# beautifulv0id/Convex-2D-GPU-Collision-Detection

Hardware: AMD Instinct MI355X
Metric: sat_pair_tests_per_s (higher is better)
Workload: dtype f32

## Files before the change

### convex-2d-gpu-collision-detection_amd/csrc/c2d_api.hip

```cpp
#include "c2d_internal.hpp"

namespace c2d {

__global__ void workspace_stamp_kernel(unsigned long long* stamp, unsigned ticket) { atomicMax(reinterpret_cast<unsigned*>(stamp), ticket); }

void workspace_stamp_behind(c2d_ctx* ctx, hipStream_t s)
{
    if (stream_is_capturing(s)) return;
    const unsigned ticket = workspace_next_ticket(ctx);
    hipLaunchKernelGGL(workspace_stamp_kernel, dim3(1), dim3(1), 0, s, ctx->d_ws_stamps + kStampOther, ticket);
    if (hipGetLastError() != hipSuccess) {
        (void)hipStreamSynchronize(s);
        (void)hipGetLastError();
        return;
    }
    ctx->ws_expect[kStampOther] = ticket;
    workspace_tickets_on(ctx, s);
}

}

extern "C" {

int c2d_version(void) { return C2D_VERSION_MAJOR * 1000 + C2D_VERSION_MINOR; }

const char* c2d_status_string(int status)
{
    switch (status) {
    case C2D_OK: return "ok";
    case C2D_ERR_INVALID_ARG: return "invalid argument";
    case C2D_ERR_HIP: return "HIP runtime error";
    case C2D_ERR_NO_DEVICE: return "no usable device";
    case C2D_ERR_NOMEM: return "out of memory";
    case C2D_ERR_UNSUPPORTED: return "unsupported argument combination";
    case C2D_ERR_DIST: return "multi-GPU (RCCL) error";
    default: return "unknown status";
    }
}

const char* c2d_last_error(const c2d_ctx* ctx) { return ctx ? ctx->last_error.c_str() : ""; }

int c2d_device_count(int* count)
{
    if (!count) return C2D_ERR_INVALID_ARG;
    int n = 0;
    if (hipGetDeviceCount(&n) != hipSuccess) { *count = 0; return C2D_ERR_NO_DEVICE; }
    *count = n;
    return C2D_OK;
}

int c2d_ctx_create(int device, c2d_ctx** out)
{
    if (!out) return C2D_ERR_INVALID_ARG;
    *out = nullptr;
    int n = 0;
    if (hipGetDeviceCount(&n) != hipSuccess || n <= 0 || device < 0 || device >= n) return C2D_ERR_NO_DEVICE;
    c2d_ctx* ctx = new (std::nothrow) c2d_ctx();
    if (!ctx) return C2D_ERR_NOMEM;
    ctx->device = device;
    if (hipGetDeviceProperties(&ctx->prop, device) != hipSuccess) { delete ctx; return C2D_ERR_NO_DEVICE; }
    if (std::strncmp(ctx->prop.gcnArchName, "gfx950", 6) != 0) { delete ctx; return C2D_ERR_NO_DEVICE; }
    c2d::DeviceGuard g(device);
    if (!g.ok) { delete ctx; return C2D_ERR_NO_DEVICE; }
    if (hipMalloc(&ctx->d_counters, 64) != hipSuccess || hipMalloc(&ctx->d_count_words, c2d::kWorkspaceBytes) != hipSuccess ||
        hipMemset(ctx->d_count_words, 0, c2d::kWorkspaceBytes) != hipSuccess || hipMalloc(&ctx->d_bins, 32 * sizeof(float)) != hipSuccess ||
        hipHostMalloc(reinterpret_cast<void**>(&ctx->h_pinned), 64, hipHostMallocDefault) != hipSuccess ||
        hipHostMalloc(reinterpret_cast<void**>(&ctx->h_async_err), 64, hipHostMallocMapped) != hipSuccess ||
        hipHostGetDevicePointer(reinterpret_cast<void**>(&ctx->d_async_err), ctx->h_async_err, 0) != hipSuccess) {
        if (ctx->d_counters) (void)hipFree(ctx->d_counters);
        if (ctx->d_count_words) (void)hipFree(ctx->d_count_words);
        if (ctx->d_bins) (void)hipFree(ctx->d_bins);
        if (ctx->h_pinned) (void)hipHostFree(ctx->h_pinned);
        if (ctx->h_async_err) (void)hipHostFree(ctx->h_async_err);
        delete ctx;
        return C2D_ERR_NOMEM;
    }
    *ctx->h_async_err = 0;
    ctx->d_count_words2 = ctx->d_count_words + c2d::kCountWordsBytes / 8;
    ctx->d_ws_stamps = ctx->d_count_words + c2d::kWorkspaceStampsOffset / 8;
    *out = ctx;
    return C2D_OK;
}

int c2d_ctx_destroy(c2d_ctx* ctx)
{
    if (!ctx) return C2D_OK;
    c2d::DeviceGuard g(ctx->device);
    for (auto& p : ctx->d_list)
        if (p) (void)hipFree(p);
    if (ctx->d_counters) (void)hipFree(ctx->d_counters);
    if (ctx->d_count_words) (void)hipFree(ctx->d_count_words);
    if (ctx->ws_probe_stream) (void)hipStreamDestroy(ctx->ws_probe_stream);
    if (ctx->h_ws_block) (void)hipHostFree(ctx->h_ws_block);
    if (ctx->d_bins) (void)hipFree(ctx->d_bins);
    if (ctx->d_scratch) (void)hipFree(ctx->d_scratch);
    c2d_host_pipe_free(ctx->host_pipe);
    if (ctx->h_pinned) (void)hipHostFree(ctx->h_pinned);
    if (ctx->h_async_err) (void)hipHostFree(ctx->h_async_err);
    delete ctx;
    return C2D_OK;
}

int c2d_ctx_info_sized(const c2d_ctx* ctx, c2d_device_info* out, size_t out_bytes)
{
    if (!ctx || !out || out_bytes == 0) return C2D_ERR_INVALID_ARG;
    c2d_device_info di;
    std::memset(&di, 0, sizeof di);
    if (ctx->prop.name[0]) std::snprintf(di.name, sizeof di.name, "%s", ctx->prop.name);
    else std::snprintf(di.name, sizeof di.name, "gfx950 device (the runtime reports no marketing name)");
    std::snprintf(di.arch, sizeof di.arch, "%s", ctx->prop.gcnArchName);
    di.device = ctx->device;
    di.compute_units = ctx->prop.multiProcessorCount;
    di.wavefront_size = ctx->prop.warpSize;
    di.lds_bytes_per_cu = (int)ctx->prop.maxSharedMemoryPerMultiProcessor;
    di.hbm_bytes = ctx->prop.totalGlobalMem;
    if (hipDeviceGetPCIBusId(di.pci_bus_id, (int)sizeof di.pci_bus_id, ctx->device) != hipSuccess) {
        (void)hipGetLastError();
        di.pci_bus_id[0] = 0;
    }
    std::memcpy(out, &di, out_bytes < sizeof di ? out_bytes : sizeof di);
    return C2D_OK;
// ... 118 lines not shown
```

### convex-2d-gpu-collision-detection_amd/csrc/c2d_internal.hpp

```cpp
#pragma once

#include <dlfcn.h>
#include <hip/hip_runtime.h>

#include <cstdio>
#include <cstring>
#include <string>

#include "../../include/c2d.h"
#include "c2d_count.hpp"

struct c2d_host_pipe;
void c2d_host_pipe_free(c2d_host_pipe* p);

struct c2d_ctx {
    int device = 0;
    hipDeviceProp_t prop{};
    uint32_t* d_list[2] = {nullptr, nullptr};
    size_t list_capacity = 0;
    uint32_t* d_counters = nullptr;
    unsigned long long* d_count_words = nullptr;
    unsigned long long* d_count_words2 = nullptr;
    unsigned long long* d_ws_stamps = nullptr;
    float* d_bins = nullptr;
    c2d_host_pipe* host_pipe = nullptr;
    void* d_scratch = nullptr;
    size_t scratch_bytes = 0;
    uint32_t* h_pinned = nullptr;
    uint32_t* h_async_err = nullptr;
    uint32_t* d_async_err = nullptr;
    hipStream_t ws_stream = nullptr;
    unsigned long long ws_stream_id = 0;
    bool ws_ticket_pending = false;
    bool ws_outstanding = false;
    unsigned ws_ticket = 0;
    unsigned ws_expect[c2d::kStampSlots] = {};
    hipStream_t ws_probe_stream = nullptr;
    unsigned long long* h_ws_block = nullptr;
    mutable std::string last_error;
};

#define C2D_ASYNC_ERR_POLY_K 1u
#define C2D_ASYNC_ERR_PAIR_INDEX 2u


namespace c2d {

inline int fail_hip(const c2d_ctx* ctx, hipError_t e, const char* what, const char* file, int line)
{
    if (ctx) {
        char buf[512];
        std::snprintf(buf, sizeof buf, "%s failed: %s (%s:%d)", what, hipGetErrorString(e), file, line);
        ctx->last_error = buf;
    }
    return C2D_ERR_HIP;
}

inline int fail_arg(const c2d_ctx* ctx, const char* msg)
{
    if (ctx) ctx->last_error = msg;
    return C2D_ERR_INVALID_ARG;
}

#define C2D_HIP(ctx, call)                                                        \
    do {                                                                          \
        hipError_t e__ = (call);                                                  \
        if (e__ != hipSuccess) return c2d::fail_hip(ctx, e__, #call, __FILE__, __LINE__); \
    } while (0)

#define C2D_LAUNCH_CHECK(ctx)                                                     \
    do {                                                                          \
        hipError_t e__ = hipGetLastError();                                       \
        if (e__ != hipSuccess) {                                                  \
            c2d::workspace_launch_failed(ctx);                                    \
            return c2d::fail_hip(ctx, e__, "kernel launch", __FILE__, __LINE__);  \
        }                                                                         \
        c2d::workspace_launch_ok(ctx);                                            \
    } while (0)

struct DeviceGuard {
    int prev = -1;
    bool ok = true;
    explicit DeviceGuard(int dev)
    {
        if (hipGetDevice(&prev) != hipSuccess) prev = -1;
        if (prev != dev) ok = hipSetDevice(dev) == hipSuccess;
    }
    ~DeviceGuard()
    {
        if (prev >= 0) (void)hipSetDevice(prev);
    }
};

constexpr int kMaxGrid = 1 << 24;

inline bool stream_is_capturing(hipStream_t s)
{
    hipStreamCaptureStatus st = hipStreamCaptureStatusNone;
    if (hipStreamIsCapturing(s, &st) != hipSuccess) { (void)hipGetLastError(); return false; }
    return st != hipStreamCaptureStatusNone;
}

constexpr unsigned long long kUnknownStreamId = ~0ull;
using StreamGetIdFn = hipError_t (*)(hipStream_t, unsigned long long*);
inline StreamGetIdFn stream_get_id_fn()
{
    static const StreamGetIdFn fn = [] {
        void* h = dlopen("libamdhip64.so.7", RTLD_NOLOAD | RTLD_NOW);
        void* sym = h ? dlsym(h, "hipStreamGetId") : nullptr;
        if (!sym) sym = dlsym(RTLD_DEFAULT, "hipStreamGetId");
        return reinterpret_cast<StreamGetIdFn>(sym);
    }();
    return fn;
}
inline unsigned long long stream_identity(hipStream_t s)
{
    const StreamGetIdFn fn = stream_get_id_fn();
    unsigned long long id = 0;
    if (!fn) return kUnknownStreamId;
    if (fn(s, &id) != hipSuccess) { (void)hipGetLastError(); return kUnknownStreamId; }
    return id;
}

inline bool workspace_same_stream(c2d_ctx* ctx, hipStream_t s)
{
    if (ctx->ws_stream != s) return false;
    if (ctx->ws_stream_id != kUnknownStreamId) return stream_identity(s) == ctx->ws_stream_id;
    return true;
}

inline hipStream_t forgotten_stream() { return reinterpret_cast<hipStream_t>(~static_cast<uintptr_t>(0)); }

inline int workspace_acquire(c2d_ctx* ctx, hipStream_t s, bool uses)
{
    ctx->ws_ticket_pending = false;
    if (!uses || !ctx->ws_outstanding) return C2D_OK;
    if (workspace_same_stream(ctx, s)) return C2D_OK;
    if (stream_is_capturing(s)) return C2D_OK;
    if (!ctx->ws_probe_stream) {
        hipError_t e = hipStreamCreateWithFlags(&ctx->ws_probe_stream, hipStreamNonBlocking);
        if (e == hipSuccess) e = hipHostMalloc(reinterpret_cast<void**>(&ctx->h_ws_block), kWorkspaceBytes, hipHostMallocDefault);
        if (e != hipSuccess) {
            if (ctx->ws_probe_stream) { (void)hipStreamDestroy(ctx->ws_probe_stream); ctx->ws_probe_stream = nullptr; }
            return fail_hip(ctx, e, "workspace guard set-up", __FILE__, __LINE__);
        }
    }
    hipError_t e = hipMemcpyAsync(ctx->h_ws_block, ctx->d_count_words, kWorkspaceBytes, hipMemcpyDeviceToHost, ctx->ws_probe_stream);
// ... 109 lines not shown
```

### convex-2d-gpu-collision-detection_amd/csrc/c2d_mc.hip

```cpp
#include "c2d_internal.hpp"
#include "c2d_math.hpp"

namespace c2d {

#ifdef C2D_MC_STATS
__device__ unsigned long long c2d_mc_stats_words[12];
#define C2D_MC_STAT(i, v)                                                                                     \
    do {                                                                                                      \
        const unsigned long long v__ = (unsigned long long)(v);                                               \
        if ((threadIdx.x & 63) == 0 && v__) atomicAdd(&c2d_mc_stats_words[i], v__);                           \
    } while (0)
#else
#define C2D_MC_STAT(i, v) do { } while (0)
#endif

}

#include "c2d_mc_core.hpp"

#ifdef C2D_MC_CLOCK
namespace c2d {
C2D_MC_CLOCK_WORDS(c2d_mc_clock_pair);
C2D_MC_CLOCK_WORDS(c2d_mc_clock_scenes);
}
// ... 363 lines not shown
#endif
constexpr bool kParkAdaptive = C2D_MC_PARK_ADAPTIVE != 0;
C2D_DEV Scene adaptive_scene(const Scene& sc, WaveQueue& q)
{
    if constexpr (kParkAdaptive) return park_scene(sc, q);
    else return park_exact(sc, q);
}

template <bool PARKED>
C2D_DEV uint32_t wave_count_hits_plain(const Scene& sc, uint64_t seed, uint64_t scene_id, uint64_t begin, uint32_t count, const WaveQueue& wq)
{
    const uint32_t lane = threadIdx.x & 63;
    uint32_t hits = 0;
#pragma nounroll
    for (uint32_t i = 0; i < count; i += 64) {
        const bool live = i + lane < count;
        const uint64_t s = begin + i + lane;
        const uint32_t j = (uint32_t)s & 3u;
        const U4 b0 = philox_draw_block(seed, scene_id, s >> 2, 0), b1 = philox_draw_block(seed, scene_id, s >> 2, 1);
        const U4 b2 = philox_draw_block(seed, scene_id, s >> 2, 2u + (j >> 1));
        float dx, dy, o[8];
        sample_centre(sc, u4_word(b0, (int)j), u4_word(b1, (int)j), dx, dy);
        const Scene ev = load_exact(load_eval<PARKED>(sc, wq), wq);
        float hx, hy, sn, cs;
        sample_shape(ev, (j & 1u) ? b2.z : b2.x, (j & 1u) ? b2.w : b2.y, seed, scene_id, s, hx, hy, sn, cs);
        rect_from_half_extents(hx, hy, cs, sn, dx, dy, o);
        hits += (uint32_t)__popcll(__ballot(live && rect_collide(ev.robot, o)));
    }
    return hits;
}

template <bool PARKED>
struct RectPolicy {
    using Scene = c2d::Scene;
    using Queue = WaveQueue;
    static C2D_DEV bool centre_pretest(const Scene& sc, const Queue&, float dx, float dy, unsigned long long& miss_m) { return c2d::centre_pretest(sc, dx, dy, miss_m); }
    static C2D_DEV uint32_t evaluate(const Scene& sc, Queue& wq, uint32_t w2r, uint32_t w2a, float dx, float dy, uint64_t seed, uint64_t scene_id, uint64_t sample,
                                     unsigned long long live_m)
    {
        return evaluate_samples<PARKED>(sc, wq, w2r, w2a, dx, dy, seed, scene_id, sample, live_m);
    }
    static C2D_DEV uint32_t plain(const Scene& sc, uint64_t seed, uint64_t scene_id, uint64_t begin, uint32_t count, const Queue& wq)
    {
        return wave_count_hits_plain<PARKED>(sc, seed, scene_id, begin, count, wq);
    }
    static C2D_DEV uint32_t finish(const Scene&, Queue&) { return 0u; }
};

struct PairArgs {
    float robot_w, robot_h, px, py;
    Pose pose;
    StdDev sd;
    uint64_t seed, scene_id, sample_begin, n_samples;
    uint32_t chunk;
};

#ifndef C2D_MC_PAIR_WAVES
#define C2D_MC_PAIR_WAVES 5
#endif
__global__ __launch_bounds__(kMcBlock, C2D_MC_PAIR_WAVES) void mc_pair_kernel(PairArgs A, unsigned long long* __restrict__ d_hits)
{
    __shared__ WaveQueue s_queue[kWavesPerBlock];
    const uint32_t wave = __builtin_amdgcn_readfirstlane(threadIdx.x >> 6);
    const Scene sc = park_exact(make_scene(A.robot_w, A.robot_h, A.px, A.py, A.pose, A.sd), s_queue[wave]);
    const uint64_t n_chunks = (A.n_samples + A.chunk - 1) / A.chunk;
    unsigned long long total = 0;
    C2D_MC_CLOCK_START();
    for (uint64_t ch = (uint64_t)blockIdx.x * kWavesPerBlock + wave; ch < n_chunks; ch += (uint64_t)gridDim.x * kWavesPerBlock) {
        const uint64_t off = ch * A.chunk;
        const uint64_t left = A.n_samples - off;
        const uint32_t count = left < A.chunk ? (uint32_t)left : A.chunk;
        total += wave_count_hits<RectPolicy<false>>(sc, A.seed, A.scene_id, A.sample_begin + off, count, s_queue[wave]);
    }
    C2D_MC_CLOCK_STOP(c2d_mc_clock_pair);
    if ((threadIdx.x & 63) == 0 && total) atomicAdd(d_hits, total);
}

struct ScenesArgs {
    const Pose* poses;
    const StdDev* std_devs;
    const PositionWithVarAndPoseIdx* scenes;
    AdaptiveState* state;
    uint32_t* lists[2];
    uint32_t num_poses, num_std_devs;
    float robot_w, robot_h;
    uint64_t seed, scene_id_base;
    ScheduleArgs sched;
    uint32_t* hits;
    uint32_t burst_steps;
    uint32_t n_bins;
    float bins[16], acc[16];
    uint32_t* n_used;
    PoseCPVarAndPoseIdx* rows;
};

struct RectBuilder {
    using Args = ScenesArgs;
    using Policy = RectPolicy<kParkAdaptive>;
#ifdef C2D_MC_CLOCK
    static C2D_DEV unsigned long long* clock_words() { return c2d_mc_clock_scenes; }
#endif
    static C2D_DEV Scene scene(const Args& A, const PositionWithVarAndPoseIdx& row, WaveQueue& q)
    {
        uint32_t pi = (uint32_t)(int)row.pose_idx, vi = (uint32_t)(int)row.var_idx;
        pi = pi < A.num_poses ? pi : A.num_poses - 1;
        vi = vi < A.num_std_devs ? vi : A.num_std_devs - 1;
        return adaptive_scene(make_scene(A.robot_w, A.robot_h, row.x, row.y, A.poses[pi], A.std_devs[vi]), q);
    }
};

__global__ void mc_scenes_init_kernel(AdaptiveState* state, uint32_t n_scenes)
{
    AdaptiveState init{};
    init.n_active = n_scenes;
    init.identity = 1;
    *state = init;
}

#ifndef C2D_MC_ADV_WAVES
#define C2D_MC_ADV_WAVES 7
#endif
template <bool BURST>
__global__ __launch_bounds__(kMcBlock, C2D_MC_ADV_WAVES) void mc_scenes_advance_kernel(ScenesArgs A) { mc_scenes_advance_body<BURST, RectBuilder>(A); }

__global__ __launch_bounds__(256) void mc_scenes_decide_kernel(DecideArgs A)
{
    const uint32_t n_active = A.state->n_active;
    if (n_active == 0) return;
// ... 106 lines not shown
                                 float* __restrict__ out1)
{
    const size_t stride = (size_t)gridDim.x * blockDim.x;
    for (size_t i = (size_t)blockIdx.x * blockDim.x + threadIdx.x; i < n; i += stride) {
        const uint32_t bits = in[i];
        const float x = __uint_as_float(bits);
        float a = 0.0f, b = 0.0f;
        switch (fn) {
        case C2D_MATH_LOG: a = log_(x); break;
        case C2D_MATH_SINCOS: sincos_(x, a, b); break;
        case C2D_MATH_SINCOS_U32: sincos_u32(bits, a, b); break;
        case C2D_MATH_SQRT: a = sqrt_normal_range(x); break;
        case C2D_MATH_BOX_MULLER: box_muller(bits, ~bits * 2654435761u, a, b); break;
        default: break;
        }
        out0[i] = a;
        if (out1) out1[i] = b;
    }
}

constexpr uint64_t kSceneDomain = 0x5ce9e5a3c0117de5ull;

__global__ void sample_scenes_kernel(const Pose* __restrict__ poses, uint32_t num_poses,
                                     const StdDev* __restrict__ std_devs, uint32_t num_std_devs, float r_offset,
                                     float spread, uint64_t seed, uint64_t scene_id_base, size_t n,
                                     PositionWithVarAndPoseIdx* __restrict__ scenes)
{
    const size_t stride = (size_t)gridDim.x * blockDim.x;
    for (size_t g = (size_t)blockIdx.x * blockDim.x + threadIdx.x; g < n; g += stride) {
        const U4 a = philox_block(seed ^ kSceneDomain, scene_id_base + g, 0, 0);
        const U4 b = philox_block(seed ^ kSceneDomain, scene_id_base + g, 0, 1);
        const uint32_t pose_idx = a.x % num_poses;
        const uint32_t sd_idx = a.y % num_std_devs;
        const Pose pose = poses[pose_idx];
        const StdDev sd = std_devs[sd_idx];
        const float u = fma_((float)a.z, 0x1p-32f, 0x1p-33f);
        const float theta = (float)((double)u * 2 * 3.14159265358979323846);
        float nrm, unused;
        box_muller(b.x, b.y, nrm, unused);
        const float shift = nrm * ((sd.y + sd.x) / 2) * spread;
        float st, ct;
        sincos_(theta, st, ct);
        const double bx = ((double)(pose.width / 2 + r_offset) + 2.35 + (double)sd.x) + (double)shift;
        const double by = ((double)(pose.height / 2 + r_offset) + 2.35 + (double)sd.y) + (double)shift;
        PositionWithVarAndPoseIdx row;
        row.x = (float)((double)ct * bx);
        row.y = (float)((double)st * by);
        row.var_idx = (float)sd_idx;
        row.pose_idx = (float)pose_idx;
        scenes[g] = row;
    }
}

void launch_mc_scenes_init(hipStream_t s, AdaptiveState* state, uint32_t n_scenes)
{
    hipLaunchKernelGGL(mc_scenes_init_kernel, dim3(1), dim3(1), 0, s, state, n_scenes);
}

void launch_mc_scenes_decide(hipStream_t s, unsigned blocks, const DecideArgs& D)
{
    hipLaunchKernelGGL(mc_scenes_decide_kernel, dim3(blocks), dim3(256), 0, s, D);
}

int ensure_scene_lists(c2d_ctx* ctx, size_t n)
{
    if (ctx->list_capacity >= n) return C2D_OK;
    for (auto& p : ctx->d_list) {
        if (p) (void)hipFree(p);
        p = nullptr;
    }
    ctx->list_capacity = 0;
    for (auto& p : ctx->d_list) {
        hipError_t e = hipMalloc(&p, n * sizeof(uint32_t));
        if (e != hipSuccess) { ctx->last_error = "c2d_mc_scenes: workspace allocation failed"; return C2D_ERR_NOMEM; }
    }
    ctx->list_capacity = n;
    return C2D_OK;
}

}

using namespace c2d;

extern "C" {

int c2d_math_eval(c2d_ctx* ctx, int fn, const uint32_t* d_in_bits, size_t n, float* d_out0, float* d_out1, c2d_stream stream)
{
    if (!ctx) return C2D_ERR_INVALID_ARG;
    if (n == 0) return C2D_OK;
    if (!d_in_bits || !d_out0 || fn < C2D_MATH_LOG || fn > C2D_MATH_BOX_MULLER) return fail_arg(ctx, "c2d_math_eval: bad argument");
    DeviceGuard g(ctx->device);
    hipLaunchKernelGGL(math_eval_kernel, dim3(grid_for(n, 256, ctx->prop.multiProcessorCount * 8)), dim3(256), 0,
                       (hipStream_t)stream, fn, d_in_bits, n, d_out0, d_out1);
    C2D_LAUNCH_CHECK(ctx);
    return C2D_OK;
}

int c2d_philox_normals(c2d_ctx* ctx, uint64_t seed, uint64_t scene_id, uint64_t sample_begin, size_t n,
                       float* d_normals, uint32_t* d_raw, c2d_stream stream)
{
    if (!ctx) return C2D_ERR_INVALID_ARG;
    if (n == 0) return C2D_OK;
    if (!d_normals) return fail_arg(ctx, "c2d_philox_normals: NULL output");
    DeviceGuard g(ctx->device);
    hipLaunchKernelGGL(philox_normals_kernel, dim3(grid_for(n, 256, ctx->prop.multiProcessorCount * 8)), dim3(256), 0,
                       (hipStream_t)stream, seed, scene_id, sample_begin, n, d_normals, d_raw);
    C2D_LAUNCH_CHECK(ctx);
    return C2D_OK;
}

int c2d_mc_pair(c2d_ctx* ctx, float robot_w, float robot_h, const Position* pos, const Pose* pose,
                const StdDev* std_dev, uint64_t seed, uint64_t scene_id, uint64_t sample_begin, uint64_t n_samples,
                unsigned long long* d_hits, c2d_stream stream)
{
    if (!ctx) return C2D_ERR_INVALID_ARG;
    if (!pos || !pose || !std_dev || !d_hits) return fail_arg(ctx, "c2d_mc_pair: NULL argument");
    if (n_samples == 0) return C2D_OK;
    if (sample_begin + n_samples < sample_begin || sample_begin + n_samples > (1ull << 62))
        return fail_arg(ctx, "c2d_mc_pair: sample range overflows the 2^62-sample stream");
    PairArgs A;
    A.robot_w = robot_w; A.robot_h = robot_h; A.px = pos->x; A.py = pos->y;
    A.pose = *pose; A.sd = *std_dev;
    A.seed = seed; A.scene_id = scene_id; A.sample_begin = sample_begin; A.n_samples = n_samples;
    const uint64_t target_waves = (uint64_t)ctx->prop.multiProcessorCount * 32;
    uint64_t chunk = (n_samples + target_waves - 1) / target_waves;
    chunk = ((chunk + 255) / 256) * 256;
    if (chunk < 256) chunk = 256;
    if (chunk > 8192) chunk = 8192;
    A.chunk = (uint32_t)chunk;
    const uint64_t n_chunks = (n_samples + chunk - 1) / chunk;
    uint64_t blocks = (n_chunks + kWavesPerBlock - 1) / kWavesPerBlock;
    const uint64_t max_blocks = (uint64_t)ctx->prop.multiProcessorCount * 256 / kWavesPerBlock;
    if (blocks > max_blocks) blocks = max_blocks;
    DeviceGuard g(ctx->device);
    hipLaunchKernelGGL(mc_pair_kernel, dim3((unsigned)blocks), dim3(kMcBlock), 0, (hipStream_t)stream, A, d_hits);
    C2D_LAUNCH_CHECK(ctx);
    return C2D_OK;
}

int c2d_mc_scenes(c2d_ctx* ctx, const c2d_mc_scenes_args* a, c2d_stream stream)
{
    if (!ctx) return C2D_ERR_INVALID_ARG;
    if (!a) return fail_arg(ctx, "c2d_mc_scenes: NULL args");
    if (a->n_scenes != 0 && (!a->d_poses || a->num_poses == 0)) {
        if (a->total_samples) *a->total_samples = 0;
        if (a->iterations) *a->iterations = 0;
        return fail_arg(ctx, a->d_poses ? "c2d_mc_scenes: empty pose / std_dev table" : "c2d_mc_scenes: NULL argument");
    }
    ScenesArgs A;
    A.poses = a->d_poses; A.num_poses = a->num_poses; A.robot_w = a->robot_w; A.robot_h = a->robot_h;
    return run_adaptive(ctx, a, stream, A, [](bool burst, unsigned blocks, const ScenesArgs& args, hipStream_t s) {
        if (burst) hipLaunchKernelGGL(mc_scenes_advance_kernel<true>, dim3(blocks), dim3(kMcBlock), 0, s, args);
        else hipLaunchKernelGGL(mc_scenes_advance_kernel<false>, dim3(blocks), dim3(kMcBlock), 0, s, args);
    }, "c2d_mc_scenes");
}

int c2d_sample_scenes(c2d_ctx* ctx, const Pose* d_poses, uint32_t num_poses, const StdDev* d_std_devs,
                      uint32_t num_std_devs, float robot_w, float robot_h, float spread, uint64_t seed,
                      uint64_t scene_id_base, size_t n_scenes, PositionWithVarAndPoseIdx* d_scenes, c2d_stream stream)
{
    if (!ctx) return C2D_ERR_INVALID_ARG;
    if (n_scenes == 0) return C2D_OK;
    if (!d_poses || !d_std_devs || !d_scenes || num_poses == 0 || num_std_devs == 0)
        return fail_arg(ctx, "c2d_sample_scenes: NULL / empty argument");
    DeviceGuard g(ctx->device);
    const float r_offset = (robot_w + robot_h) / 4;
    hipLaunchKernelGGL(sample_scenes_kernel, dim3(grid_for(n_scenes, 256, ctx->prop.multiProcessorCount * 8)), dim3(256), 0,
                       (hipStream_t)stream, d_poses, num_poses, d_std_devs, num_std_devs, r_offset, spread, seed,
                       scene_id_base, n_scenes, d_scenes);
    C2D_LAUNCH_CHECK(ctx);
    return C2D_OK;
}

#ifdef C2D_MC_CLOCK
int c2d_debug_mc_clock(c2d_ctx* ctx, int which, unsigned long long out[4], int reset)
{
    if (!ctx || !out || which < 0 || which > 1) return C2D_ERR_INVALID_ARG;
    DeviceGuard g(ctx->device);
    C2D_HIP(ctx, hipDeviceSynchronize());
    const unsigned long long zero[4] = {};
    if (which == 0) {
        C2D_HIP(ctx, hipMemcpyFromSymbol(out, HIP_SYMBOL(c2d_mc_clock_pair), 4 * sizeof(unsigned long long)));
        if (reset) C2D_HIP(ctx, hipMemcpyToSymbol(HIP_SYMBOL(c2d_mc_clock_pair), zero, sizeof zero));
    } else {
        C2D_HIP(ctx, hipMemcpyFromSymbol(out, HIP_SYMBOL(c2d_mc_clock_scenes), 4 * sizeof(unsigned long long)));
        if (reset) C2D_HIP(ctx, hipMemcpyToSymbol(HIP_SYMBOL(c2d_mc_clock_scenes), zero, sizeof zero));
    }
    return C2D_OK;
// ... 38 lines not shown
```

### convex-2d-gpu-collision-detection_amd/csrc/c2d_mc_core.hpp

```cpp
#pragma once

#include "c2d_internal.hpp"
#include "c2d_math.hpp"
#include "c2d_wave.hpp"

#ifndef C2D_MC_STAT
#define C2D_MC_STAT(i, v) do { } while (0)
#endif

#ifdef C2D_MC_CLOCK
#define C2D_MC_CLOCK_WORDS(name) __device__ unsigned long long name[4]
struct McClockStamp {
    unsigned long long c0, r0;
    __device__ __forceinline__ McClockStamp() : c0(__builtin_amdgcn_s_memtime()), r0(__builtin_amdgcn_s_memrealtime()) {}
    __device__ __forceinline__ void stop(unsigned long long* words) const
    {
        const unsigned long long c1 = __builtin_amdgcn_s_memtime(), r1 = __builtin_amdgcn_s_memrealtime();
        if ((threadIdx.x & 63) == 0) {
            atomicAdd(&words[0], c1 - c0);
            atomicAdd(&words[1], r1 - r0);
            atomicAdd(&words[2], 1ull);
        }
    }
};
// ... 200 lines not shown
        if (cn) {
            wave_lds_sync();
            const uint32_t take = cn < 64 ? cn : 64;
            const bool live = lane < take;
            const unsigned long long live_m = take >= 64 ? ~0ull : (1ull << take) - 1;
            const uint2 e = q.cand[cn - take + (live ? lane : 0)];
            wave_lds_sync();
            cn -= take;
            const uint64_t s = begin + e.y;
            const U4 a = philox_draw_block(seed, scene_id, s >> 2, 1);
            const uint32_t jj = (uint32_t)s & 3u;
            const uint32_t aw = jj == 0 ? a.x : (jj == 1 ? a.y : (jj == 2 ? a.z : a.w));
            float dx, dy;
            C2D_MC_STAT(4, take);
            sample_centre(sc, e.x, aw, dx, dy);
            unsigned long long miss_m;
            const bool miss = P::centre_pretest(sc, wq, dx, dy, miss_m);
            const bool undecided = live && !miss;
            const unsigned long long m = live_m & ~miss_m;
            if (undecided) {
                const uint32_t slot = un + __builtin_amdgcn_mbcnt_hi((uint32_t)(m >> 32), __builtin_amdgcn_mbcnt_lo((uint32_t)m, 0u));
                q.und_c[slot] = make_float2(dx, dy);
                q.und_idx[slot] = e.y;
            }
            un += (uint32_t)__popcll(m);
        }
        if (un >= 64 || (drained && cn == 0 && un)) hits += evaluate_queued<P>(sc, wq, q.und_c, q.und_idx, un, un < 64 ? un : 64u, seed, scene_id, begin);
        if (drained && cn == 0 && un == 0) break;
    }
    return hits;
}
#endif

template <class P>
C2D_DEV uint32_t wave_count_hits(const typename P::Scene& sc, uint64_t seed, uint64_t scene_id, uint64_t begin, uint32_t count,
                                 typename P::Queue& q)
{
    C2D_MC_STAT(0, count);
    if (!sc.tame()) return P::plain(sc, seed, scene_id, begin, count, q);
#ifndef C2D_MC_NO_PRETEST
    if (sc.use_x0 && sc.x0 < kFarX0) {
        C2D_MC_STAT(1, count);
        const uint32_t h = wave_count_hits_far<P>(sc, seed, scene_id, begin, count, q) + P::finish(sc, q);
        C2D_MC_STAT(7, h);
        return h;
    }
#endif
    C2D_MC_STAT(2, count);
    const uint32_t h = wave_count_hits_near<P>(sc, seed, scene_id, begin, count, q) + P::finish(sc, q);
    C2D_MC_STAT(7, h);
    return h;
}

struct AdaptiveState {
    uint32_t n_active;
    uint32_t next_count;
    uint32_t n_samples;
    uint32_t iter;
    uint32_t ticket;
    uint32_t list_sel;
    uint32_t identity;
    uint32_t burst_steps;
    unsigned long long total_samples;
};

struct ScheduleArgs {
    uint32_t small_batch, large_batch, switch_at, max_samples;
    uint32_t want_waves;
    uint32_t min_chunk;
};

C2D_DEV uint32_t batch_of(const ScheduleArgs& S, uint32_t n_samples)
{
    return n_samples < S.switch_at ? S.small_batch : S.large_batch;
}

C2D_DEV float calc_slack(uint32_t n, uint32_t k)
{
    if (k == n || k == 0) {
        return (float)(0x1.d82d33932720dp+1 / (double)n);
    }
    const float z = 1.96f;
    const float kf = (float)k;
    const float kk = (float)((uint64_t)k * (uint64_t)k);
    return z / (float)n * __builtin_sqrtf(kf - kk / (float)n);
}

C2D_DEV int get_bin(float p, const float* bins, uint32_t n_bins)
{
    int bin = 0;
    for (uint32_t i = 0; i + 1 < n_bins; i++)
        if (p >= bins[i] && p <= bins[i + 1]) bin = (int)i;
    return bin;
}

template <bool BURST, class B>
C2D_DEV void mc_scenes_advance_body(const typename B::Args& A)
{
    using P = typename B::Policy;
    __shared__ typename P::Queue s_queue[kWavesPerBlock];
    const uint32_t n_active = A.state->n_active;
    if (n_active == 0) return;
    const uint32_t n_start = A.state->n_samples;
    if (n_start >= A.sched.max_samples) return;
    const uint32_t n_batch = batch_of(A.sched, n_start);
    const uint32_t* active = A.state->identity ? nullptr : A.lists[A.state->list_sel];
// ... 180 lines not shown
```

### convex-2d-gpu-collision-detection_amd/csrc/c2d_mc_poly.hip

```cpp
#include <type_traits>

#include "c2d_internal.hpp"
#include "c2d_math.hpp"

#ifdef C2D_MC_STATS
namespace c2d {
__device__ unsigned long long c2d_mc_poly_stats_words[12];
}
#define C2D_MC_STAT(i, v)                                                                                     \
    do {                                                                                                      \
        const unsigned long long v__ = (unsigned long long)(v);                                               \
        if ((threadIdx.x & 63) == 0 && v__) atomicAdd(&c2d::c2d_mc_poly_stats_words[i], v__);                 \
    } while (0)
#endif
#include "c2d_mc_core.hpp"

namespace c2d {

#ifndef C2D_MC_POLY_PLAIN_PAIR_LOOP
#define C2D_MC_POLY_PLAIN_PAIR_LOOP 0
#endif
constexpr int KM = C2D_POLY_KMAX;
#ifndef C2D_MC_POLY_IN_PLACE
#define C2D_MC_POLY_IN_PLACE 48
// ... 354 lines not shown
        C2D_MC_STAT(6, __popcll(alive));
        uint32_t n = q.n_surv;
        if ((alive >> (threadIdx.x & 63)) & 1ull) {
            const uint32_t slot = n + __builtin_amdgcn_mbcnt_hi((uint32_t)(alive >> 32), __builtin_amdgcn_mbcnt_lo((uint32_t)alive, 0u));
            q.surv_a[slot] = make_float4(dx, dy, c, s);
            q.surv_b[slot] = make_float2(fx, fy);
        }
        n += (uint32_t)__popcll(alive);
        uint32_t hits = 0;
        if (n >= 64) hits = evaluate_survivors(sc, q, n, 64);
        wave_lds_sync();
        if ((threadIdx.x & 63) == 0) q.n_surv = n;
        wave_lds_sync();
        return hits;
    }
    static C2D_DEV uint32_t finish(const Scene& sc, Queue& q)
    {
        uint32_t n = q.n_surv;
        if (n == 0) return 0u;
        uint32_t hits = 0;
        while (n) hits += evaluate_survivors(sc, q, n, n < 64 ? n : 64u);
        wave_lds_sync();
        if ((threadIdx.x & 63) == 0) q.n_surv = 0;
        wave_lds_sync();
        return hits;
    }
    static C2D_DEV uint32_t plain(const Scene& sc, uint64_t seed, uint64_t scene_id, uint64_t begin, uint32_t count, const Queue& q)
    {
        const uint32_t lane = threadIdx.x & 63;
        uint32_t hits = 0;
#pragma nounroll
        for (uint32_t i = 0; i < count; i += 64) {
            const uint32_t left = count - i;
            const unsigned long long live_m = left >= 64 ? ~0ull : (1ull << left) - 1;
            const uint64_t sm = begin + i + lane;
            const uint32_t j = (uint32_t)sm & 3u;
            const U4 b0 = philox_draw_block(seed, scene_id, sm >> 2, 0), b1 = philox_draw_block(seed, scene_id, sm >> 2, 1);
            const U4 b2 = philox_draw_block(seed, scene_id, sm >> 2, 2u + (j >> 1));
            float dx, dy, c, s, fx, fy;
            sample_centre(sc, u4_word(b0, (int)j), u4_word(b1, (int)j), dx, dy);
            poly_sample_shape(sc, (j & 1u) ? b2.z : b2.x, (j & 1u) ? b2.w : b2.y, seed, scene_id, sm, c, s, fx, fy);
            bool final;
            hits += (uint32_t)__popcll(poly_sample_stage_any<true, 0>(sc, q, dx, dy, c, s, fx, fy, live_m, final));
        }
        return hits;
    }
};

struct PolyPairArgs {
    c2d_polygon robot, obstacle;
    float px, py, theta;
    StdDev sd;
    uint64_t seed, scene_id, sample_begin, n_samples;
    uint32_t chunk;
};

#ifndef C2D_MC_POLY_WAVES
#define C2D_MC_POLY_WAVES 5
#endif
#ifdef C2D_MC_CLOCK
C2D_MC_CLOCK_WORDS(c2d_mc_clock_poly_pair);
C2D_MC_CLOCK_WORDS(c2d_mc_clock_poly);
#endif
__global__ __launch_bounds__(kMcBlock, C2D_MC_POLY_WAVES) void mc_poly_pair_kernel(PolyPairArgs A, unsigned long long* __restrict__ d_hits)
{
    __shared__ PolyQueue s_queue[kWavesPerBlock];
    const uint32_t wave = __builtin_amdgcn_readfirstlane(threadIdx.x >> 6);
    const uint32_t l = threadIdx.x & 15;
    const PolyScene sc = build_poly_scene(lane_pick(A.robot.x, l), lane_pick(A.robot.y, l), (int)A.robot.k, A.px, A.py, A.theta, lane_pick(A.obstacle.x, l),
                                          lane_pick(A.obstacle.y, l), (int)A.obstacle.k, A.sd, s_queue[wave]);
    const uint64_t n_chunks = (A.n_samples + A.chunk - 1) / A.chunk;
    unsigned long long total = 0;
    C2D_MC_CLOCK_START();
    for (uint64_t ch = (uint64_t)blockIdx.x * kWavesPerBlock + wave; ch < n_chunks; ch += (uint64_t)gridDim.x * kWavesPerBlock) {
        const uint64_t off = ch * A.chunk;
        const uint64_t left = A.n_samples - off;
        const uint32_t count = left < A.chunk ? (uint32_t)left : A.chunk;
        total += wave_count_hits<PolyPolicy>(sc, A.seed, A.scene_id, A.sample_begin + off, count, s_queue[wave]);
    }
    C2D_MC_CLOCK_STOP(c2d_mc_clock_poly_pair);
    if ((threadIdx.x & 63) == 0 && total) atomicAdd(d_hits, total);
}

struct PolyScenesArgs {
    const StdDev* std_devs;
    const PositionWithVarAndPoseIdx* scenes;
    AdaptiveState* state;
    uint32_t* lists[2];
    uint32_t num_std_devs;
    uint64_t seed, scene_id_base;
    ScheduleArgs sched;
    uint32_t* hits;
    uint32_t burst_steps;
    uint32_t n_bins;
    float bins[16], acc[16];
    uint32_t* n_used;
    PoseCPVarAndPoseIdx* rows;
    const c2d_poly_pose* poly_poses;
    uint32_t num_poly_poses;
    c2d_polygon robot;
    uint32_t* async_err;
};

struct PolyBuilder {
    using Args = PolyScenesArgs;
    using Policy = PolyPolicy;
#ifdef C2D_MC_CLOCK
    static C2D_DEV unsigned long long* clock_words() { return c2d_mc_clock_poly; }
#endif
    static C2D_DEV PolyScene scene(const Args& A, const PositionWithVarAndPoseIdx& row, PolyQueue& q)
    {
        uint32_t pi = (uint32_t)(int)row.pose_idx, vi = (uint32_t)(int)row.var_idx;
        pi = pi < A.num_poly_poses ? pi : A.num_poly_poses - 1;
        vi = vi < A.num_std_devs ? vi : A.num_std_devs - 1;
        const c2d_poly_pose* pp = A.poly_poses + pi;
        const uint32_t l = threadIdx.x & 15;
        const float theta = pp->theta, ovx = pp->obstacle.x[l], ovy = pp->obstacle.y[l];
        uint32_t kb = pp->obstacle.k, ka = A.robot.k;
        if (kb < 1 || kb > (uint32_t)KM) {
            if ((threadIdx.x & 63) == 0) __hip_atomic_fetch_or(A.async_err, C2D_ASYNC_ERR_POLY_K, __ATOMIC_RELAXED, __HIP_MEMORY_SCOPE_SYSTEM);
            kb = kb < 1 ? 1u : (uint32_t)KM;
        }
        ka = ka < 1 ? 1u : (ka > (uint32_t)KM ? (uint32_t)KM : ka);
        return build_poly_scene(lane_pick(A.robot.x, l), lane_pick(A.robot.y, l), (int)ka, row.x, row.y, theta, ovx, ovy, (int)kb, A.std_devs[vi], q);
    }
};

template <bool BURST>
__global__ __launch_bounds__(kMcBlock, C2D_MC_POLY_WAVES) void mc_poly_scenes_advance_kernel(PolyScenesArgs A) { mc_scenes_advance_body<BURST, PolyBuilder>(A); }

}

using namespace c2d;

namespace {

const char* polygon_fault(const c2d_polygon* p)
{
    if (!p) return "NULL polygon";
    if (p->k < 1 || p->k > (uint32_t)C2D_POLY_KMAX) return "polygon vertex count outside 1..C2D_POLY_KMAX";
    return nullptr;
}

c2d_polygon tidy(const c2d_polygon& p)
{
    c2d_polygon o = p;
    for (uint32_t k = p.k; k < (uint32_t)C2D_POLY_KMAX; k++) o.x[k] = o.y[k] = 0.0f;
    return o;
}

}

extern "C" {

int c2d_mc_poly_pair(c2d_ctx* ctx, const c2d_polygon* robot, const Position* pos, float robot_theta, const c2d_polygon* obstacle, const StdDev* std_dev,
                     uint64_t seed, uint64_t scene_id, uint64_t sample_begin, uint64_t n_samples, unsigned long long* d_hits, c2d_stream stream)
{
    if (!ctx) return C2D_ERR_INVALID_ARG;
    if (!robot || !pos || !obstacle || !std_dev || !d_hits) return fail_arg(ctx, "c2d_mc_poly_pair: NULL argument");
    if (const char* f = polygon_fault(robot)) return fail_arg(ctx, (std::string("c2d_mc_poly_pair: robot: ") + f).c_str());
    if (const char* f = polygon_fault(obstacle)) return fail_arg(ctx, (std::string("c2d_mc_poly_pair: obstacle: ") + f).c_str());
    if (n_samples == 0) return C2D_OK;
    if (sample_begin + n_samples < sample_begin || sample_begin + n_samples > (1ull << 62))
        return fail_arg(ctx, "c2d_mc_poly_pair: sample range overflows the 2^62-sample stream");
    PolyPairArgs A;
    A.robot = tidy(*robot); A.obstacle = tidy(*obstacle);
    A.px = pos->x; A.py = pos->y; A.theta = robot_theta; A.sd = *std_dev;
    A.seed = seed; A.scene_id = scene_id; A.sample_begin = sample_begin; A.n_samples = n_samples;
    const uint64_t target_waves = (uint64_t)ctx->prop.multiProcessorCount * 32;
    uint64_t chunk = (n_samples + target_waves - 1) / target_waves;
    chunk = ((chunk + 255) / 256) * 256;
    if (chunk < 256) chunk = 256;
    if (chunk > 8192) chunk = 8192;
    A.chunk = (uint32_t)chunk;
    const uint64_t n_chunks = (n_samples + chunk - 1) / chunk;
    uint64_t blocks = (n_chunks + kWavesPerBlock - 1) / kWavesPerBlock;
    const uint64_t max_blocks = (uint64_t)ctx->prop.multiProcessorCount * 256 / kWavesPerBlock;
    if (blocks > max_blocks) blocks = max_blocks;
    DeviceGuard g(ctx->device);
    hipLaunchKernelGGL(mc_poly_pair_kernel, dim3((unsigned)blocks), dim3(kMcBlock), 0, (hipStream_t)stream, A, d_hits);
    C2D_LAUNCH_CHECK(ctx);
    return C2D_OK;
}

int c2d_mc_poly_scenes(c2d_ctx* ctx, const c2d_mc_poly_scenes_args* a, c2d_stream stream)
{
    if (!ctx) return C2D_ERR_INVALID_ARG;
    if (!a) return fail_arg(ctx, "c2d_mc_poly_scenes: NULL args");
    const c2d_mc_scenes_args* b = &a->base;
    if (b->n_scenes != 0) {
        const char* why = nullptr;
        if (!a->d_poly_poses) why = "c2d_mc_poly_scenes: NULL argument";
        else if (a->num_poly_poses == 0) why = "c2d_mc_poly_scenes: empty pose / std_dev table";
        else if (polygon_fault(a->robot)) why = "c2d_mc_poly_scenes: robot: NULL or vertex count outside 1..C2D_POLY_KMAX";
        if (why) {
            if (b->total_samples) *b->total_samples = 0;
            if (b->iterations) *b->iterations = 0;
            return fail_arg(ctx, why);
        }
    }
    PolyScenesArgs A;
    A.poly_poses = a->d_poly_poses; A.num_poly_poses = a->num_poly_poses;
    if (a->robot) A.robot = tidy(*a->robot);
    A.async_err = ctx->d_async_err;
    return run_adaptive(ctx, b, stream, A, [](bool burst, unsigned blocks, const PolyScenesArgs& args, hipStream_t s) {
        if (burst) hipLaunchKernelGGL(mc_poly_scenes_advance_kernel<true>, dim3(blocks), dim3(kMcBlock), 0, s, args);
        else hipLaunchKernelGGL(mc_poly_scenes_advance_kernel<false>, dim3(blocks), dim3(kMcBlock), 0, s, args);
    }, "c2d_mc_poly_scenes");
}

#ifdef C2D_MC_STATS
int c2d_debug_mc_poly_stats(c2d_ctx* ctx, unsigned long long out[12], int reset)
{
    if (!ctx || !out) return C2D_ERR_INVALID_ARG;
    DeviceGuard g(ctx->device);
    C2D_HIP(ctx, hipDeviceSynchronize());
    C2D_HIP(ctx, hipMemcpyFromSymbol(out, HIP_SYMBOL(c2d_mc_poly_stats_words), 12 * sizeof(unsigned long long)));
    if (reset) {
        const unsigned long long zero[12] = {};
        C2D_HIP(ctx, hipMemcpyToSymbol(HIP_SYMBOL(c2d_mc_poly_stats_words), zero, sizeof zero));
    }
    return C2D_OK;
}
#endif

#ifdef C2D_MC_CLOCK
int c2d_debug_mc_poly_clock(c2d_ctx* ctx, int which, unsigned long long out[4], int reset)
{
    if (!ctx || !out || which < 0 || which > 1) return C2D_ERR_INVALID_ARG;
    DeviceGuard g(ctx->device);
    C2D_HIP(ctx, hipDeviceSynchronize());
    const unsigned long long zero[4] = {};
    if (which == 0) {
// ... 12 lines not shown
```

Before: 96.42 billion.

## Split Monte Carlo pair sample range into contiguous per-wave spans sized by occupancy

Replaces the grid-stride chunk loop in the rect and polygon pair kernels with a static split. Each wave receives one contiguous span of 256-sample iterations, and the number of waves is set from occupancy-queried resident waves times a split factor. A smaller block of four waves is used, and per-block hit totals are reduced in shared memory before a single atomic. The aim is to cut per-chunk loop overhead, tail imbalance and atomic traffic. The cost is an occupancy query at context creation and possible load imbalance when samples vary in cost.

```diff
diff --git a/convex-2d-gpu-collision-detection_amd/csrc/c2d_api.hip b/convex-2d-gpu-collision-detection_amd/csrc/c2d_api.hip
--- a/convex-2d-gpu-collision-detection_amd/csrc/c2d_api.hip
+++ b/convex-2d-gpu-collision-detection_amd/csrc/c2d_api.hip
@@ -66,7 +66,8 @@
         hipMemset(ctx->d_count_words, 0, c2d::kWorkspaceBytes) != hipSuccess || hipMalloc(&ctx->d_bins, 32 * sizeof(float)) != hipSuccess ||
         hipHostMalloc(reinterpret_cast<void**>(&ctx->h_pinned), 64, hipHostMallocDefault) != hipSuccess ||
         hipHostMalloc(reinterpret_cast<void**>(&ctx->h_async_err), 64, hipHostMallocMapped) != hipSuccess ||
-        hipHostGetDevicePointer(reinterpret_cast<void**>(&ctx->d_async_err), ctx->h_async_err, 0) != hipSuccess) {
+        hipHostGetDevicePointer(reinterpret_cast<void**>(&ctx->d_async_err), ctx->h_async_err, 0) != hipSuccess ||
+        c2d::mc_pair_ask_resident_waves(ctx) != hipSuccess || c2d::mc_poly_pair_ask_resident_waves(ctx) != hipSuccess) {
         if (ctx->d_counters) (void)hipFree(ctx->d_counters);
         if (ctx->d_count_words) (void)hipFree(ctx->d_count_words);
         if (ctx->d_bins) (void)hipFree(ctx->d_bins);
diff --git a/convex-2d-gpu-collision-detection_amd/csrc/c2d_internal.hpp b/convex-2d-gpu-collision-detection_amd/csrc/c2d_internal.hpp
--- a/convex-2d-gpu-collision-detection_amd/csrc/c2d_internal.hpp
+++ b/convex-2d-gpu-collision-detection_amd/csrc/c2d_internal.hpp
@@ -37,6 +37,7 @@
     unsigned ws_expect[c2d::kStampSlots] = {};
     hipStream_t ws_probe_stream = nullptr;
     unsigned long long* h_ws_block = nullptr;
+    uint32_t mc_resident_waves[2] = {0, 0};
     mutable std::string last_error;
 };
 
@@ -93,6 +94,9 @@
 };
 
 constexpr int kMaxGrid = 1 << 24;
+
+hipError_t mc_pair_ask_resident_waves(c2d_ctx* ctx);
+hipError_t mc_poly_pair_ask_resident_waves(c2d_ctx* ctx);
 
 inline bool stream_is_capturing(hipStream_t s)
 {
diff --git a/convex-2d-gpu-collision-detection_amd/csrc/c2d_mc.hip b/convex-2d-gpu-collision-detection_amd/csrc/c2d_mc.hip
--- a/convex-2d-gpu-collision-detection_amd/csrc/c2d_mc.hip
+++ b/convex-2d-gpu-collision-detection_amd/csrc/c2d_mc.hip
@@ -439,28 +439,30 @@
     Pose pose;
     StdDev sd;
     uint64_t seed, scene_id, sample_begin, n_samples;
-    uint32_t chunk;
+    SpanSplit split;
 };
 
+#ifdef C2D_MC_ROUND_SPLIT
+#define C2D_MC_PAIR_SPLIT C2D_MC_ROUND_SPLIT
+#elif !defined(C2D_MC_PAIR_SPLIT)
+#define C2D_MC_PAIR_SPLIT 4
+#endif
 #ifndef C2D_MC_PAIR_WAVES
 #define C2D_MC_PAIR_WAVES 5
 #endif
-__global__ __launch_bounds__(kMcBlock, C2D_MC_PAIR_WAVES) void mc_pair_kernel(PairArgs A, unsigned long long* __restrict__ d_hits)
-{
-    __shared__ WaveQueue s_queue[kWavesPerBlock];
+__global__ __launch_bounds__(kMcPairBlock, C2D_MC_PAIR_WAVES) void mc_pair_kernel(PairArgs A, unsigned long long* __restrict__ d_hits)
+{
+    __shared__ WaveQueue s_queue[kMcPairBlockWaves];
     const uint32_t wave = __builtin_amdgcn_readfirstlane(threadIdx.x >> 6);
-    const Scene sc = park_exact(make_scene(A.robot_w, A.robot_h, A.px, A.py, A.pose, A.sd), s_queue[wave]);
-    const uint64_t n_chunks = (A.n_samples + A.chunk - 1) / A.chunk;
+    const uint32_t w = blockIdx.x * kMcPairBlockWaves + wave;
     unsigned long long total = 0;
-    C2D_MC_CLOCK_START();
-    for (uint64_t ch = (uint64_t)blockIdx.x * kWavesPerBlock + wave; ch < n_chunks; ch += (uint64_t)gridDim.x * kWavesPerBlock) {
-        const uint64_t off = ch * A.chunk;
-        const uint64_t left = A.n_samples - off;
-        const uint32_t count = left < A.chunk ? (uint32_t)left : A.chunk;
-        total += wave_count_hits<RectPolicy<false>>(sc, A.seed, A.scene_id, A.sample_begin + off, count, s_queue[wave]);
-    }
-    C2D_MC_CLOCK_STOP(c2d_mc_clock_pair);
-    if ((threadIdx.x & 63) == 0 && total) atomicAdd(d_hits, total);
+    if (w < A.split.waves) {
+        const Scene sc = park_exact(make_scene(A.robot_w, A.robot_h, A.px, A.py, A.pose, A.sd), s_queue[wave]);
+        C2D_MC_CLOCK_START();
+        total = wave_count_span<RectPolicy<false>>(sc, A.seed, A.scene_id, A.sample_begin, A.n_samples, A.split, w, s_queue[wave]);
+        C2D_MC_CLOCK_STOP(c2d_mc_clock_pair);
+    }
+    block_add_hits(total, d_hits);
 }
 
 struct ScenesArgs {
@@ -673,6 +675,16 @@
     }
 }
 
+hipError_t mc_pair_ask_resident_waves(c2d_ctx* ctx)
+{
+    int per_cu = 0;
+    const hipError_t e = hipOccupancyMaxActiveBlocksPerMultiprocessor(&per_cu, mc_pair_kernel, kMcPairBlock, 0);
+    if (e != hipSuccess) return e;
+    if (per_cu < 1) return hipErrorInvalidValue;
+    ctx->mc_resident_waves[0] = (uint32_t)per_cu * kMcPairBlockWaves * (uint32_t)ctx->prop.multiProcessorCount;
+    return hipSuccess;
+}
+
 void launch_mc_scenes_init(hipStream_t s, AdaptiveState* state, uint32_t n_scenes)
 {
     hipLaunchKernelGGL(mc_scenes_init_kernel, dim3(1), dim3(1), 0, s, state, n_scenes);
@@ -743,18 +755,10 @@
     A.robot_w = robot_w; A.robot_h = robot_h; A.px = pos->x; A.py = pos->y;
     A.pose = *pose; A.sd = *std_dev;
     A.seed = seed; A.scene_id = scene_id; A.sample_begin = sample_begin; A.n_samples = n_samples;
-    const uint64_t target_waves = (uint64_t)ctx->prop.multiProcessorCount * 32;
-    uint64_t chunk = (n_samples + target_waves - 1) / target_waves;
-    chunk = ((chunk + 255) / 256) * 256;
-    if (chunk < 256) chunk = 256;
-    if (chunk > 8192) chunk = 8192;
-    A.chunk = (uint32_t)chunk;
-    const uint64_t n_chunks = (n_samples + chunk - 1) / chunk;
-    uint64_t blocks = (n_chunks + kWavesPerBlock - 1) / kWavesPerBlock;
-    const uint64_t max_blocks = (uint64_t)ctx->prop.multiProcessorCount * 256 / kWavesPerBlock;
-    if (blocks > max_blocks) blocks = max_blocks;
+    A.split = split_spans(sample_begin, n_samples, ctx->mc_resident_waves[0], C2D_MC_PAIR_SPLIT);
+    const unsigned blocks = (A.split.waves + kMcPairBlockWaves - 1) / kMcPairBlockWaves;
     DeviceGuard g(ctx->device);
-    hipLaunchKernelGGL(mc_pair_kernel, dim3((unsigned)blocks), dim3(kMcBlock), 0, (hipStream_t)stream, A, d_hits);
+    hipLaunchKernelGGL(mc_pair_kernel, dim3(blocks), dim3(kMcPairBlock), 0, (hipStream_t)stream, A, d_hits);
     C2D_LAUNCH_CHECK(ctx);
     return C2D_OK;
 }
diff --git a/convex-2d-gpu-collision-detection_amd/csrc/c2d_mc_core.hpp b/convex-2d-gpu-collision-detection_amd/csrc/c2d_mc_core.hpp
--- a/convex-2d-gpu-collision-detection_amd/csrc/c2d_mc_core.hpp
+++ b/convex-2d-gpu-collision-detection_amd/csrc/c2d_mc_core.hpp
@@ -276,6 +276,66 @@
     return h;
 }
 
+#ifndef C2D_MC_PAIR_BLOCK_WAVES
+#define C2D_MC_PAIR_BLOCK_WAVES 4
+#endif
+constexpr int kMcPairBlockWaves = C2D_MC_PAIR_BLOCK_WAVES;
+constexpr int kMcPairBlock = 64 * kMcPairBlockWaves;
+constexpr uint64_t kMcPieceIters = 1ull << 23;
+
+struct SpanSplit {
+    uint64_t q;
+    uint32_t r;
+    uint32_t waves;
+};
+
+inline SpanSplit split_spans(uint64_t sample_begin, uint64_t n_samples, uint32_t resident_waves, uint32_t split)
+{
+    const uint64_t iters = ((sample_begin & 3) + n_samples + 255) / 256;
+    const uint64_t most = (uint64_t)resident_waves * split;
+    SpanSplit s;
+    s.waves = (uint32_t)(iters < most ? iters : most);
+    s.q = iters / s.waves;
+    s.r = (uint32_t)(iters % s.waves);
+    return s;
+}
+
+template <class P>
+C2D_DEV unsigned long long wave_count_span(const typename P::Scene& sc, uint64_t seed, uint64_t scene_id, uint64_t sample_begin, uint64_t n_samples,
+                                           const SpanSplit& S, uint32_t w, typename P::Queue& q)
+{
+    const uint64_t base = sample_begin & 3, origin = sample_begin - base, end_pos = base + n_samples;
+    uint64_t it = (uint64_t)w * S.q + (w < S.r ? w : S.r);
+    const uint64_t it_end = it + S.q + (w < S.r ? 1u : 0u);
+    unsigned long long total = 0;
+    while (it < it_end) {
+        const uint64_t step = it_end - it < kMcPieceIters ? it_end - it : kMcPieceIters;
+        uint64_t p0 = it * 256, p1 = (it + step) * 256;
+        p0 = p0 < base ? base : p0;
+        p1 = p1 > end_pos ? end_pos : p1;
+        total += wave_count_hits<P>(sc, seed, scene_id, origin + p0, (uint32_t)(p1 - p0), q);
+        it += step;
+    }
+    return total;
+}
+
+C2D_DEV void block_add_hits(unsigned long long total, unsigned long long* d_hits)
+{
+    if constexpr (kMcPairBlockWaves == 1) {
+        if ((threadIdx.x & 63) == 0 && total) atomicAdd(d_hits, total);
+    } else {
+        __shared__ unsigned long long s_total[kMcPairBlockWaves];
+        if ((threadIdx.x & 63) == 0) s_total[threadIdx.x >> 6] = total;
+        __syncthreads();
+        if (threadIdx.x == 0) {
+            unsigned long long sum = 0;
+#pragma unroll
+            for (int k = 0; k < kMcPairBlockWaves; k++) sum += s_total[k];
+            if (sum) atomicAdd(d_hits, sum);
+        }
+    }
+}
+
 struct AdaptiveState {
     uint32_t n_active;
     uint32_t next_count;
diff --git a/convex-2d-gpu-collision-detection_amd/csrc/c2d_mc_poly.hip b/convex-2d-gpu-collision-detection_amd/csrc/c2d_mc_poly.hip
--- a/convex-2d-gpu-collision-detection_amd/csrc/c2d_mc_poly.hip
+++ b/convex-2d-gpu-collision-detection_amd/csrc/c2d_mc_poly.hip
@@ -430,9 +430,14 @@
     float px, py, theta;
     StdDev sd;
     uint64_t seed, scene_id, sample_begin, n_samples;
-    uint32_t chunk;
+    SpanSplit split;
 };
 
+#ifdef C2D_MC_ROUND_SPLIT
+#define C2D_MC_POLY_PAIR_SPLIT C2D_MC_ROUND_SPLIT
+#elif !defined(C2D_MC_POLY_PAIR_SPLIT)
+#define C2D_MC_POLY_PAIR_SPLIT 8
+#endif
 #ifndef C2D_MC_POLY_WAVES
 #define C2D_MC_POLY_WAVES 5
 #endif
@@ -440,24 +445,31 @@
 C2D_MC_CLOCK_WORDS(c2d_mc_clock_poly_pair);
 C2D_MC_CLOCK_WORDS(c2d_mc_clock_poly);
 #endif
-__global__ __launch_bounds__(kMcBlock, C2D_MC_POLY_WAVES) void mc_poly_pair_kernel(PolyPairArgs A, unsigned long long* __restrict__ d_hits)
-{
-    __shared__ PolyQueue s_queue[kWavesPerBlock];
+__global__ __launch_bounds__(kMcPairBlock, C2D_MC_POLY_WAVES) void mc_poly_pair_kernel(PolyPairArgs A, unsigned long long* __restrict__ d_hits)
+{
+    __shared__ PolyQueue s_queue[kMcPairBlockWaves];
     const uint32_t wave = __builtin_amdgcn_readfirstlane(threadIdx.x >> 6);
-    const uint32_t l = threadIdx.x & 15;
-    const PolyScene sc = build_poly_scene(lane_pick(A.robot.x, l), lane_pick(A.robot.y, l), (int)A.robot.k, A.px, A.py, A.theta, lane_pick(A.obstacle.x, l),
-                                          lane_pick(A.obstacle.y, l), (int)A.obstacle.k, A.sd, s_queue[wave]);
-    const uint64_t n_chunks = (A.n_samples + A.chunk - 1) / A.chunk;
+    const uint32_t w = blockIdx.x * kMcPairBlockWaves + wave;
     unsigned long long total = 0;
-    C2D_MC_CLOCK_START();
-    for (uint64_t ch = (uint64_t)blockIdx.x * kWavesPerBlock + wave; ch < n_chunks; ch += (uint64_t)gridDim.x * kWavesPerBlock) {
-        const uint64_t off = ch * A.chunk;
-        const uint64_t left = A.n_samples - off;
-        const uint32_t count = left < A.chunk ? (uint32_t)left : A.chunk;
-        total += wave_count_hits<PolyPolicy>(sc, A.seed, A.scene_id, A.sample_begin + off, count, s_queue[wave]);
-    }
-    C2D_MC_CLOCK_STOP(c2d_mc_clock_poly_pair);
-    if ((threadIdx.x & 63) == 0 && total) atomicAdd(d_hits, total);
+    if (w < A.split.waves) {
+        const uint32_t l = threadIdx.x & 15;
+        const PolyScene sc = build_poly_scene(lane_pick(A.robot.x, l), lane_pick(A.robot.y, l), (int)A.robot.k, A.px, A.py, A.theta, lane_pick(A.obstacle.x, l),
+                                              lane_pick(A.obstacle.y, l), (int)A.obstacle.k, A.sd, s_queue[wave]);
+        C2D_MC_CLOCK_START();
+        total = wave_count_span<PolyPolicy>(sc, A.seed, A.scene_id, A.sample_begin, A.n_samples, A.split, w, s_queue[wave]);
+        C2D_MC_CLOCK_STOP(c2d_mc_clock_poly_pair);
+    }
+    block_add_hits(total, d_hits);
+}
+
+hipError_t mc_poly_pair_ask_resident_waves(c2d_ctx* ctx)
+{
+    int per_cu = 0;
+    const hipError_t e = hipOccupancyMaxActiveBlocksPerMultiprocessor(&per_cu, mc_poly_pair_kernel, kMcPairBlock, 0);
+    if (e != hipSuccess) return e;
+    if (per_cu < 1) return hipErrorInvalidValue;
+    ctx->mc_resident_waves[1] = (uint32_t)per_cu * kMcPairBlockWaves * (uint32_t)ctx->prop.multiProcessorCount;
+    return hipSuccess;
 }
 
 struct PolyScenesArgs {
@@ -545,18 +557,10 @@
     A.robot = tidy(*robot); A.obstacle = tidy(*obstacle);
     A.px = pos->x; A.py = pos->y; A.theta = robot_theta; A.sd = *std_dev;
     A.seed = seed; A.scene_id = scene_id; A.sample_begin = sample_begin; A.n_samples = n_samples;
-    const uint64_t target_waves = (uint64_t)ctx->prop.multiProcessorCount * 32;
-    uint64_t chunk = (n_samples + target_waves - 1) / target_waves;
-    chunk = ((chunk + 255) / 256) * 256;
-    if (chunk < 256) chunk = 256;
-    if (chunk > 8192) chunk = 8192;
-    A.chunk = (uint32_t)chunk;
-    const uint64_t n_chunks = (n_samples + chunk - 1) / chunk;
-    uint64_t blocks = (n_chunks + kWavesPerBlock - 1) / kWavesPerBlock;
-    const uint64_t max_blocks = (uint64_t)ctx->prop.multiProcessorCount * 256 / kWavesPerBlock;
-    if (blocks > max_blocks) blocks = max_blocks;
+    A.split = split_spans(sample_begin, n_samples, ctx->mc_resident_waves[1], C2D_MC_POLY_PAIR_SPLIT);
+    const unsigned blocks = (A.split.waves + kMcPairBlockWaves - 1) / kMcPairBlockWaves;
     DeviceGuard g(ctx->device);
-    hipLaunchKernelGGL(mc_poly_pair_kernel, dim3((unsigned)blocks), dim3(kMcBlock), 0, (hipStream_t)stream, A, d_hits);
+    hipLaunchKernelGGL(mc_poly_pair_kernel, dim3(blocks), dim3(kMcPairBlock), 0, (hipStream_t)stream, A, d_hits);
     C2D_LAUNCH_CHECK(ctx);
     return C2D_OK;
 }
```

After: 96.48 billion, median of 3. About the same (+0.1%).
